# rknightion/iq-to-audio

Hardware: AMD Instinct MI355X
Metric: complex IQ MS/s end-to-end (ingest->48 kHz audio) (higher is better)
Workload: dtype i8; 1 GPU; BASELINE config 2: synthetic 60 s @ 10 MS/s int16 I/Q, 1 NFM channel, +25 kHz, bw 12.5 kHz, D=104, 6401 taps, chunk 4194304; frames_per_gpu=600000000, parallelism=1 independent capture(s), one per GPU; RCCL gather of 48 kHz audio only, audio_samples_48k=2879996, mix_sign=1, settle_steps=55

## Files before the change

iq-to-audio_amd/csrc/channelize_ring.hip:

```cpp
#include "mfma_common.h"

#include <atomic>
#include <mutex>
#include <cmath>
#include <type_traits>

namespace iqa {

typedef __attribute__((address_space(3))) void ring_lds_t;

constexpr int RG_WAVES = 8;

constexpr int RG_MAX_KS = 16;
constexpr int RG_ROWS_MAX_KS_C = 11;
constexpr int RG_W = 512;
constexpr int RG_GUARD = 64;
constexpr int RG_AS = RG_W + RG_GUARD;
constexpr int RG_ACC_BYTES = 2 * RG_AS * 8;
constexpr int RG_EMIT_WAVE = 2;
constexpr int RG_EMIT_LAG = 3;
constexpr unsigned int RG_PACE_AHEAD = 2;
constexpr int RG_PACE_SPINS = 20000;
constexpr int RG_PACE_WORDS = 16384;
constexpr int RG_PAIR_IDLE = 1 << 28;
constexpr int RG_LOADERS_MAX_KS = 13;
constexpr int RG_ROUNDS_MAX = 5;
constexpr int RG_PAIR_ROUNDS = 3;
constexpr int RG_PD = 2;

__device__ __forceinline__ void ring_dma16(const void *src, ring_lds_t *dst)
{
#if defined(__HIP_DEVICE_COMPILE__)
    __builtin_amdgcn_global_load_lds(src, dst, 16, 0, 0);
#else
    (void)src;
    (void)dst;
#endif
}

__device__ __forceinline__ unsigned lds_addr(const void *p)
{
    return static_cast<unsigned>(reinterpret_cast<size_t>((__attribute__((address_space(3))) const void *)p));
}

template <int KS, bool ROWS, bool U8 = false, bool PAIR = false>
struct RingGeo {
    static_assert(ROWS || !U8, "uint8 captures use row-staged slots");
    static_assert(!PAIR || (!ROWS && !U8), "lane pairs: contiguous slots only");
    static constexpr int TPR = PAIR ? 1 : 2;
    static constexpr int ACCS = PAIR ? 2 : 1;
    static constexpr int KBYTES = U8 ? 32 : 64;
    static constexpr int PITCH = KBYTES * KS + 16;
    static constexpr bool PADDED = KS <= 13;
    static constexpr int NI = 2 * KS + 1;
    static constexpr int UNITS_ROW = PITCH / 16;
    static constexpr int NI_ROWS = (32 * UNITS_ROW + 63) / 64;
    static constexpr int SLOT_RAW = ROWS ? (32 * PITCH > 1024 * NI_ROWS ? 32 * PITCH : 1024 * NI_ROWS) : 1024 * NI;
    static constexpr bool LOADERS = (!PAIR && (ROWS || KS <= RG_LOADERS_MAX_KS)) || (PAIR && KS <= 13);
    static constexpr bool SPLIT = LOADERS && !U8;
    static constexpr int PLANE_PITCH = 32 * KS + 16;
    static constexpr int SPLIT_F = PAIR ? 3 : 2;
    static constexpr int NLOADERS = SPLIT ? 4 : (LOADERS ? 2 : 0);
    static constexpr int SLOT = SPLIT ? 64 * PLANE_PITCH : SLOT_RAW;
    static constexpr int NDMA = ROWS ? NI_ROWS : (LOADERS ? NI : KS + 1);
    static constexpr int FIT = (160 * 1024 - ACCS * RG_ACC_BYTES) / (TPR * SLOT);
    static constexpr int RMAX = 63 / NDMA + 2;
    static constexpr int R0 = FIT < RMAX ? FIT : RMAX;
    static constexpr int RCAP = PAIR ? RG_PAIR_ROUNDS : RG_ROUNDS_MAX;
    static constexpr int R = SPLIT ? 2 : R0 > RCAP ? RCAP : (R0 < 2 ? 2 : R0);
    static constexpr int THREADS = (RG_WAVES + NLOADERS) * kWave;
    static constexpr int LDS_BYTES = R * TPR * SLOT + ACCS * RG_ACC_BYTES;
    static_assert(LDS_BYTES <= 160 * 1024, "ring + window exceed LDS");
    static_assert((R - 2) * NDMA <= 63, "vmcnt is a 6-bit counter");
};

struct RingCtx {
    char *smem;
    int *s_acc;
    const char *stream0;
    long long tile_bytes, i0, m0;
    int tiles, rounds, cnt, lane_off, rt, cp, col, h, lane;
    int row_units, pitch_units;
    int tshift;
    int half_last;
};

__device__ __forceinline__ int ring_src_off(int idx, int lane, int row_units, int pitch_units)
{
    const int q = 64 * idx + lane;
    int r = q / pitch_units;
    int u = q - r * pitch_units;
    if (r > 31) {
        r = 31;
        u = row_units - 1;
    }
    return (r * row_units + min(u, row_units - 1)) * 16;
}

struct RingEmit {
    double wc, ws;
};

struct RingEmitRegs {
    double v_re, v_im;
    double2 pr;
    int i;
};

template <bool ACC64, bool EARLY>
__device__ __forceinline__ void ring_emit_load(const MfmaArgs &a, const RingCtx &c, int k, RingEmitRegs &g)
{
    const int pos = 64 * k + 1 + c.lane;
    g.i = pos - MF_Q;
    const int s = pos & (RG_W - 1);
    if constexpr (ACC64) {
        long long *acc = reinterpret_cast<long long *>(c.s_acc);
        long long sr = acc[s], si = acc[RG_AS + s];
        if (s < RG_GUARD) {
            sr += acc[RG_W + s];
            si += acc[RG_AS + RG_W + s];
            acc[RG_W + s] = 0;
            acc[RG_AS + RG_W + s] = 0;
        }
        acc[s] = 0;
        acc[RG_AS + s] = 0;
        const int s2r = static_cast<int>(sr), s2i = static_cast<int>(si);
        const long long s1r = (sr - s2r) >> 32, s1i = (si - s2i) >> 32;
        g.v_re = static_cast<double>(s1r) * 256.0 + static_cast<double>(s2r);
        g.v_im = static_cast<double>(s1i) * 256.0 + static_cast<double>(s2i);
    } else {
        int *acc = c.s_acc;
        int sr = acc[s], si = acc[RG_AS + s];
        if (s < RG_GUARD) {
            sr += acc[RG_W + s];
            si += acc[RG_AS + RG_W + s];
            acc[RG_W + s] = 0;
            acc[RG_AS + RG_W + s] = 0;
        }
        acc[s] = 0;
        acc[RG_AS + s] = 0;
        g.v_re = static_cast<double>(sr);
        g.v_im = static_cast<double>(si);
    }
    g.pr = make_double2(0.0, 0.0);
    if constexpr (EARLY) {
        if (a.partial_in != nullptr && g.i >= 0 && g.i < c.cnt) g.pr = a.partial_in[c.i0 + g.i];
    }
}

template <bool EARLY>
__device__ __forceinline__ void ring_emit_store(const MfmaArgs &a, const RingCtx &c, RingEmit &e, const RingEmitRegs &g)
{
    const int i = g.i;
    if (i >= 0 && i < c.cnt) {
        double d_re = mfma_scaled_sum(g.v_re, a.c_re, a.unit);
        double d_im = mfma_scaled_sum(g.v_im, a.c_im, a.unit);
        if (a.partial_in != nullptr) {
            const double2 pr = EARLY ? g.pr : a.partial_in[c.i0 + i];
            d_re = __dadd_rn(d_re, pr.x);
            d_im = __dadd_rn(d_im, pr.y);
        }
        if (!a.finalize) {
            if (a.raw_partials)
                reinterpret_cast<int2 *>(a.partial_out)[c.i0 + i] = make_int2(static_cast<int>(g.v_re), static_cast<int>(g.v_im));
            else
                a.partial_out[c.i0 + i] = make_double2(d_re, d_im);
        } else {
            a.out[c.i0 + i] = mfma_finish(d_re, d_im, a.conj_sum, a.rotate, e.wc, e.ws, a.sc_re, a.sc_im);
        }
    }
    const double nc = e.wc * a.rot64_re - e.ws * a.rot64_im;
    e.ws = fma(e.wc, a.rot64_im, e.ws * a.rot64_re);
    e.wc = nc;
}

template <bool ACC64>
__device__ __forceinline__ void ring_emit_group(const MfmaArgs &a, const RingCtx &c, RingEmit &e, int k)
{
    RingEmitRegs g;
    ring_emit_load<ACC64, false>(a, c, k, g);
    ring_emit_store<false>(a, c, e, g);
}

template <int KS, bool ROWS, bool U8, bool PAIR = false>
__device__ __forceinline__ void ring_wait_and_barrier(int younger)
{
    using G = RingGeo<KS, ROWS, U8, PAIR>;
    constexpr int R = G::R, N = G::NDMA;
    if (R >= 5 && younger == 3) asm volatile("s_waitcnt vmcnt(%0)\n\ts_barrier" ::"n"(R >= 5 ? 3 * N : 0) : "memory");
    else if (R >= 4 && younger == 2) asm volatile("s_waitcnt vmcnt(%0)\n\ts_barrier" ::"n"(R >= 4 ? 2 * N : 0) : "memory");
    else if (R >= 3 && younger == 1) asm volatile("s_waitcnt vmcnt(%0)\n\ts_barrier" ::"n"(R >= 3 ? N : 0) : "memory");
    else asm volatile("s_waitcnt vmcnt(0)\n\ts_barrier" ::: "memory");
}

template <int KS, bool ACC64>
__device__ __forceinline__ void ring_loader(const MfmaArgs &a, const RingCtx &c)
{
    using G = RingGeo<KS, true, true>;
    constexpr int R = G::R, SLOT = G::SLOT;
    const int cp = c.cp;
    int soff[G::NI_ROWS];
    const int row_bytes = static_cast<int>(c.tile_bytes >> 5);
#pragma unroll
    for (int i = 0; i < G::NI_ROWS; ++i) {
        const int q = 64 * i + c.lane;
        int r = q / G::UNITS_ROW;
        int u = q - r * G::UNITS_ROW;
        if (r > 31) {
            r = 31;
            u = G::UNITS_ROW - 2;
        }
        soff[i] = r * row_bytes + min(u, G::UNITS_ROW - 2) * 16;
    }
    auto issue_tile = [&](int tile, int slot) {
        const char *src = c.stream0 + static_cast<long long>(min(tile, c.tiles - 1)) * c.tile_bytes;
        char *dst = c.smem + (slot * 2 + cp) * SLOT;
#pragma unroll
        for (int i = 0; i < G::NI_ROWS; ++i)
            ring_dma16(src + soff[i], (ring_lds_t *)(dst + i * 1024));
    };
#pragma unroll
    for (int rr = 0; rr < R - 1; ++rr) issue_tile(2 * rr + cp, rr);
    RingEmit em{1.0, 0.0};
    double st_re = a.rot64_re * a.rot64_re - a.rot64_im * a.rot64_im, st_im = 2.0 * a.rot64_re * a.rot64_im;
    if (a.finalize && a.rotate) {
        const unsigned long long m = static_cast<unsigned long long>(c.m0 + (64 * cp + 1 + c.lane - MF_Q));
        const unsigned long long ph = a.rot_base + m * a.rot_step;
        sincospi(2.0 * (static_cast<double>(ph >> 11) * (1.0 / 9007199254740992.0)), &em.ws, &em.wc);
    }
    MfmaArgs a2 = a;
    a2.rot64_re = st_re;
    a2.rot64_im = st_im;
    int slot = 0;
    for (int r = 0; r < c.rounds; ++r) {
        ring_wait_and_barrier<KS, true, true>(min(R - 2, c.rounds - 1 - r));
        if (r + R - 1 < c.rounds) issue_tile(2 * (r + R - 1) + cp, (slot == 0) ? R - 1 : slot - 1);
        if (r >= RG_EMIT_LAG && ((r - RG_EMIT_LAG) & 1) == cp) {
            asm volatile("" ::: "memory");
            ring_emit_group<ACC64>(a2, c, em, r - RG_EMIT_LAG);
            asm volatile("" ::: "memory");
        }
        slot = (slot + 1 == R) ? 0 : slot + 1;
    }
    asm volatile("s_waitcnt vmcnt(0) lgkmcnt(0)\n\ts_barrier" ::: "memory");
    const int k_last = (c.cnt + 62) >> 6;
    for (int k = max(c.rounds - RG_EMIT_LAG, 0); k <= k_last; ++k)
        if ((k & 1) == cp) ring_emit_group<ACC64>(a2, c, em, k);
}

struct __attribute__((packed, aligned(4))) ring_raw16 {
    int x, y, z, w;
};

template <int KS, bool ACC64, bool ROWS, int HALF, bool PAIR = false>
__device__ __forceinline__ void ring_loader_split(const MfmaArgs &a, const RingCtx &c)
{
    constexpr bool EMITTER = PAIR ? HALF < 2 : HALF == 0;
    constexpr bool UNEVEN = !PAIR && KS >= 12;
    constexpr int P0 = KS >= 12 ? KS - 2 : KS;
    constexpr int STRIDE = PAIR ? RingGeo<KS, ROWS, false, PAIR>::NLOADERS : 2;
    constexpr int NP = UNEVEN ? (HALF ? 2 * KS - P0 : P0) : (2 * KS + STRIDE - 1) / STRIDE;
    auto piece = [](int j) { return UNEVEN ? (HALF ? P0 + j : j) : STRIDE * j + HALF; };
    using G = RingGeo<KS, ROWS, false, PAIR>;
    constexpr int SLOT = G::SLOT, PP = G::PLANE_PITCH, F = G::SPLIT_F;
    const int cp = c.cp;
    const int upr = ROWS ? 4 * KS : c.row_units;
    const int row_bytes = static_cast<int>(c.tile_bytes >> 5);
    constexpr bool TABLE = KS <= 8;
    int doff[TABLE ? NP : 1], soff[TABLE ? NP : 1];
    unsigned rowu[TABLE ? 1 : (NP + 1) / 2];
    if constexpr (!TABLE) {
#pragma unroll
        for (int j = 0; j < (NP + 1) / 2; ++j) rowu[j] = 0;
    }
#pragma unroll
    for (int j = 0; j < NP; ++j) {
        const int q = 64 * piece(j) + c.lane;
        const int row = q / upr, u = q - row * upr;
        if constexpr (TABLE) {
            doff[j] = row < 32 ? row * PP + 8 * u : -1;
            soff[j] = row < 32 ? row * row_bytes + 16 * u : 31 * row_bytes + 16 * (upr - 1);
        } else {
            const unsigned f = row < 32 ? static_cast<unsigned>((row << 6) | u) : static_cast<unsigned>((31 << 6) | (upr - 1) | (1 << 11));
            rowu[j >> 1] |= f << (16 * (j & 1));
        }
    }
    int4 buf[F][NP];
    auto request = [&](int round, auto set) {
        constexpr int S = decltype(set)::value;
        const char *src = c.stream0 + static_cast<long long>(PAIR ? min(round, c.rounds - 1) : min(2 * round + cp, c.tiles - 1)) * c.tile_bytes;
#pragma unroll
        for (int j = 0; j < NP; ++j) {
            int so;
            if constexpr (TABLE) so = soff[j];
            else {
                const unsigned f = rowu[j >> 1] >> (16 * (j & 1));
                so = static_cast<int>((f >> 6) & 31u) * row_bytes + 16 * static_cast<int>(f & 63u);
            }
            const ring_raw16 t = *reinterpret_cast<const ring_raw16 *>(src + so);
            buf[S][j] = make_int4(t.x, t.y, t.z, t.w);
        }
    };
    auto stage = [&](int slot, auto set) {
        constexpr int S = decltype(set)::value;
        char *hi0 = c.smem + (PAIR ? slot : slot * 2 + cp) * SLOT;
#pragma unroll
        for (int j = 0; j < NP; ++j) {
            const int4 d = buf[S][j];
            int2 hi, lo;
            hi.x = __builtin_amdgcn_perm(d.y, d.x, 0x07050301);
            hi.y = __builtin_amdgcn_perm(d.w, d.z, 0x07050301);
            lo.x = __builtin_amdgcn_perm(d.y, d.x, 0x06040200) ^ 0x80808080;
            lo.y = __builtin_amdgcn_perm(d.w, d.z, 0x06040200) ^ 0x80808080;
            int dq;
            if constexpr (TABLE) dq = doff[j];
            else {
                const unsigned f = rowu[j >> 1] >> (16 * (j & 1));
                dq = (f & 2048u) ? -1 : static_cast<int>((f >> 6) & 31u) * PP + 8 * static_cast<int>(f & 63u);
            }
            if (dq >= 0) {
                *reinterpret_cast<int2 *>(hi0 + dq) = hi;
                *reinterpret_cast<int2 *>(hi0 + 32 * PP + dq) = lo;
            }
        }
    };
    request(0, std::integral_constant<int, 0>{});
    stage(0, std::integral_constant<int, 0>{});
    request(1, std::integral_constant<int, 1 % F>{});
    request(2, std::integral_constant<int, 2 % F>{});
    if constexpr (F == 3) request(3, std::integral_constant<int, 0>{});
    static_assert(F == 2 || F == 3, "the prologue and the unrolled loop below are written for two or three rounds in flight");
    RingEmit em{1.0, 0.0};
    double st_re = a.rot64_re * a.rot64_re - a.rot64_im * a.rot64_im, st_im = 2.0 * a.rot64_re * a.rot64_im;
    if (EMITTER && a.finalize && a.rotate) {
        const unsigned long long m = static_cast<unsigned long long>(c.m0 + ((PAIR ? 0 : 64 * cp) + 1 + c.lane - MF_Q));
        const unsigned long long ph = a.rot_base + m * a.rot_step;
        sincospi(2.0 * (static_cast<double>(ph >> 11) * (1.0 / 9007199254740992.0)), &em.ws, &em.wc);
    }
    MfmaArgs a2 = a;
    if constexpr (!PAIR) {
        a2.rot64_re = st_re;
        a2.rot64_im = st_im;
    }
    auto group_of = [&](int r) {
        if constexpr (PAIR) {
            const int re = r - c.tshift, lag = 5 + cp;
            return (re >= lag && ((re - lag) & 1) == 0) ? (re - lag) >> 1 : -1;
        } else {
            return (r >= RG_EMIT_LAG && ((r - RG_EMIT_LAG) & 1) == cp) ? r - RG_EMIT_LAG : -1;
        }
    };
    constexpr bool PR_AHEAD = PAIR || KS <= 11;
    double2 pr_next = make_double2(0.0, 0.0);
    auto round_body = [&](int r, auto set) {
        asm volatile("s_waitcnt lgkmcnt(0)\n\ts_barrier" ::: "memory");
        if (r + 1 < c.rounds) stage((r + 1) & 1, set);
        const double2 pr_now = pr_next;
        if (PR_AHEAD && EMITTER && a.partial_in != nullptr) {
            const int kn = group_of(r + 1);
            if (kn >= 0) {
                const int i = 64 * kn + 1 + c.lane - MF_Q;
                pr_next = (i >= 0 && i < c.cnt) ? a.partial_in[c.i0 + i] : make_double2(0.0, 0.0);
            }
        }
        request(r + 1 + F, set);
        const int k = EMITTER ? group_of(r) : -1;
        if (k >= 0) {
            asm volatile("" ::: "memory");
            if constexpr (PR_AHEAD) {
                RingEmitRegs g;
                ring_emit_load<ACC64, false>(a2, c, k, g);
                g.pr = pr_now;
                ring_emit_store<true>(a2, c, em, g);
            } else {
                ring_emit_group<ACC64>(a2, c, em, k);
            }
            asm volatile("" ::: "memory");
        }
    };
    int r = 0;
    if constexpr (F == 3) {
        for (; r + 3 <= c.rounds; r += 3) {
            round_body(r, std::integral_constant<int, 1>{});
            round_body(r + 1, std::integral_constant<int, 2>{});
            round_body(r + 2, std::integral_constant<int, 0>{});
        }
        if (r < c.rounds) {
            round_body(r, std::integral_constant<int, 1>{});
            if (r + 1 < c.rounds) round_body(r + 1, std::integral_constant<int, 2>{});
        }
    } else {
        for (; r + 2 <= c.rounds; r += 2) {
            round_body(r, std::integral_constant<int, 1>{});
            round_body(r + 1, std::integral_constant<int, 0>{});
        }
        if (r < c.rounds) round_body(r, std::integral_constant<int, 1>{});
    }
    asm volatile("s_waitcnt vmcnt(0) lgkmcnt(0)\n\ts_barrier" ::: "memory");
    if constexpr (EMITTER) {
        const int k_last = (c.cnt + 62) >> 6;
        if constexpr (PAIR) {
            const int own = c.rounds - c.tshift, lag = 5 + cp;
            const int k_next = own > lag ? ((own - 1 - lag) >> 1) + 1 : 0;
            if (c.tshift < RG_PAIR_IDLE)
                for (int k = k_next; k <= k_last; ++k) ring_emit_group<ACC64>(a2, c, em, k);
        } else {
            for (int k = max(c.rounds - RG_EMIT_LAG, 0); k <= k_last; ++k)
                if ((k & 1) == cp) ring_emit_group<ACC64>(a2, c, em, k);
        }
    }
}

template <int KS, bool ACC64, bool ROWS, bool U8, bool ISSUER, bool EMIT, bool DEFER, bool PAIR, typename SKIPT, bool HALF = false>
__device__ __forceinline__ void ring_main(const MfmaArgs &a, const RingCtx &c, const v4i_t (&fq)[KS][2], SKIPT)
{
    constexpr int SKIP = SKIPT::value;
    using G = RingGeo<KS, ROWS, U8, PAIR>;
    constexpr int R = G::R, SLOT = G::SLOT;
    static_assert(!(ROWS && ISSUER), "row-staged slots are always fed by loader waves");
    const int RG_EMIT_LAG_PAIR = 5 + c.cp;
    const int rt = c.rt, cp = c.cp;
    int soff[(ISSUER && G::PADDED) ? KS + 1 : 1];
    if constexpr (ISSUER && G::PADDED) {
#pragma unroll
        for (int i = 0; i <= KS; ++i) soff[i] = ring_src_off(min(2 * i + (rt & 1), 2 * KS), c.lane, c.row_units, c.pitch_units);
    } else {
        soff[0] = c.lane * 16;
    }
    const int odd_kib = (rt & 1) * 1024;
    auto issue = [&](int tile, int slot, int i) {
        const char *tile0 = c.stream0 + static_cast<long long>(min(tile, (PAIR ? c.rounds : c.tiles) - 1)) * c.tile_bytes;
        char *slot0 = c.smem + (PAIR ? slot : slot * 2 + cp) * SLOT;
        const int at = (i < KS) ? odd_kib + i * 2048 : 2 * KS * 1024;
        if constexpr (ISSUER && G::PADDED) {
            ring_dma16(tile0 + soff[i], (ring_lds_t *)(slot0 + at));
        } else {
            ring_dma16(tile0 + soff[0] + at, (ring_lds_t *)(slot0 + at));
        }
    };
    if (ISSUER) {
#pragma unroll
        for (int rr = 0; rr < R - 1; ++rr)
#pragma unroll
            for (int i = 0; i <= KS; ++i) issue(PAIR ? rr : 2 * rr + cp, rr, i);
    }
    RingEmit em{1.0, 0.0};
    if (EMIT && a.finalize && a.rotate) {
        const unsigned long long m = static_cast<unsigned long long>(c.m0 + (1 + c.lane - MF_Q));
        const unsigned long long ph = a.rot_base + m * a.rot_step;
        sincospi(2.0 * (static_cast<double>(ph >> 11) * (1.0 / 9007199254740992.0)), &em.ws, &em.wc);
    }
    const v16i_t zero16 = {0, 0, 0, 0, 0, 0, 0, 0, 0, 0, 0, 0, 0, 0, 0, 0};
    auto scatter = [&](int t, const v16i_t &acc1, const v16i_t &acc2) {
        const int slot_idx = ((t * 32 + c.col + 4 * c.h + 1) & (RG_W - 1)) + (rt >> 1) * RG_AS + (rt & 1) * 32;
        if constexpr (ACC64) {
            const unsigned p = lds_addr(reinterpret_cast<long long *>(c.s_acc) + slot_idx);
#pragma unroll
            for (int q = 0; q < 16; ++q) {
                const long long comb = (static_cast<long long>(acc1[q]) << 32) + static_cast<long long>(acc2[q]);
                const int off = 8 * ((q & 3) + 8 * (q >> 2));
                asm volatile("ds_add_u64 %0, %1 offset:%2" ::"v"(p), "v"(comb), "n"(off));
            }
        } else {
            const unsigned p = lds_addr(c.s_acc + slot_idx);
#pragma unroll
            for (int q = 0; q < 16; ++q) {
                const int comb = (acc1[q] << 8) + acc2[q];
                const int off = 4 * ((q & 3) + 8 * (q >> 2));
                asm volatile("ds_add_u32 %0, %1 offset:%2" ::"v"(p), "v"(comb), "n"(off));
            }
        }
    };
    constexpr bool DEFER_ADDS = DEFER && !G::SPLIT;
    v16i_t held1 = zero16, held2 = zero16;
    int held_t = -1;
    int slot = 0;
    bool pace_on = PAIR && a.pace != nullptr && a.pace_units > 1 && c.rounds < 8000;
    for (int r = 0; r < c.rounds; ++r) {
        if (ISSUER) ring_wait_and_barrier<KS, ROWS, U8, PAIR>(min(R - 2, c.rounds - 1 - r));
        else asm volatile("s_barrier" ::: "memory");
        if constexpr (PAIR && !ISSUER && !EMIT && !DEFER) {
            if (c.rt == 3 && c.cp == 0 && pace_on && (r & 1) == 0) {
                const unsigned int mine = static_cast<unsigned int>(r >> 1);
                if (c.lane == 0) __hip_atomic_store(a.pace + a.pace_slot, (a.pace_token << 12) | mine, __ATOMIC_RELAXED, __HIP_MEMORY_SCOPE_AGENT);
                for (int spin = 0;; ++spin) {
                    unsigned int q = mine;
                    if (c.lane < a.pace_units) {
                        const unsigned int v = __hip_atomic_load(a.pace + (a.pace_slot - a.pace_slot % a.pace_units) + c.lane, __ATOMIC_RELAXED,
                                                                 __HIP_MEMORY_SCOPE_AGENT);
                        if ((v >> 12) == a.pace_token) q = v & 0xFFFu;
                    }
#pragma unroll
                    for (int o = 1; o < 16; o <<= 1) q = min(q, static_cast<unsigned int>(__shfl_xor(static_cast<int>(q), o, kWave)));
                    q = static_cast<unsigned int>(__builtin_amdgcn_readfirstlane(static_cast<int>(q)));
                    if (mine <= q + RG_PACE_AHEAD) break;
                    if (spin >= RG_PACE_SPINS) {
                        pace_on = false;
                        break;
                    }
                    __builtin_amdgcn_s_sleep(32);
                }
            }
        }
        const bool pf = ISSUER && (r + R - 1 < c.rounds);
        const int pf_tile = PAIR ? r + R - 1 : 2 * (r + R - 1) + cp;
        const int pf_slot = (slot == 0) ? R - 1 : slot - 1;
        if (pf) {
#pragma unroll
            for (int i = 0; i <= KS; ++i) issue(pf_tile, pf_slot, i);
        }
        const int re = r - c.tshift;
        const bool emit_now = EMIT && (PAIR ? (re >= RG_EMIT_LAG_PAIR && ((re - RG_EMIT_LAG_PAIR) & 1) == 0) : re >= RG_EMIT_LAG);
        RingEmitRegs eg;
        if (emit_now) {
            asm volatile("" ::: "memory");
            ring_emit_load<ACC64, true>(a, c, PAIR ? (re - RG_EMIT_LAG_PAIR) >> 1 : re - RG_EMIT_LAG, eg);
            asm volatile("" ::: "memory");
        }
        if (DEFER_ADDS && held_t >= 0) {
            scatter(held_t, held1, held2);
            held_t = -1;
        }
        bool store_pending = emit_now;
#pragma unroll
        for (int j = 0; j < 1; ++j) {
        const int t = PAIR ? re : 2 * r + cp;
        if (t >= 0 && t < c.tiles) {
            const bool store_here = store_pending;
            store_pending = false;
            const char *la = c.smem + (PAIR ? slot : slot * 2 + cp) * SLOT + c.lane_off;
            auto tile_body = [&](auto skip_low) {
                constexpr bool SKIP_LOW = decltype(skip_low)::value;
                constexpr int PD = KS < RG_PD ? KS : RG_PD;
                v16i_t acc1, acc2;
                if constexpr (U8) {
                    v4i_t du[KS];
#pragma unroll
                    for (int ks = 0; ks < PD; ++ks) du[ks] = *reinterpret_cast<const v4i_t *>(la + 32 * ks);
#pragma unroll
                    for (int ks = 0; ks < KS; ++ks) {
                        v4i_t v = du[ks];
                        v.x ^= 0x80808080;
                        v.y ^= 0x80808080;
                        v.z ^= 0x80808080;
                        v.w ^= 0x80808080;
                        if (ks + PD < KS) du[ks + PD] = *reinterpret_cast<const v4i_t *>(la + 32 * (ks + PD));
                        acc1 = __builtin_amdgcn_mfma_i32_32x32x32_i8(fq[ks][0], v, ks ? acc1 : zero16, 0, 0, 0);
                        acc2 = __builtin_amdgcn_mfma_i32_32x32x32_i8(fq[ks][1], v, ks ? acc2 : zero16, 0, 0, 0);
                    }
                } else if constexpr (G::SPLIT) {
                    v4i_t hh[KS], ll[KS];
                    constexpr bool half_last = HALF;
                    auto fetch = [&](int ks) {
                        if (ks == KS - 1 && half_last) {
                            const int2 h2 = *reinterpret_cast<const int2 *>(la - 8 * c.h + 32 * ks);
                            const int2 l2 = *reinterpret_cast<const int2 *>(la - 8 * c.h + 32 * G::PLANE_PITCH + 32 * ks);
                            hh[ks].x = h2.x;
                            hh[ks].y = h2.y;
                            ll[ks].x = l2.x;
                            ll[ks].y = l2.y;
                        } else {
                            hh[ks] = *reinterpret_cast<const v4i_t *>(la + 32 * ks);
                            ll[ks] = *reinterpret_cast<const v4i_t *>(la + 32 * G::PLANE_PITCH + 32 * ks);
                        }
                    };
#pragma unroll
                    for (int ks = 0; ks < PD; ++ks) fetch(ks);
#pragma unroll
                    for (int ks = 0; ks < KS; ++ks) {
                        const v4i_t hi = hh[ks], lo = ll[ks];
                        if (ks + PD < KS) fetch(ks + PD);
                        if (ks == KS - 1 && half_last) {
                            auto pack = [](int x, int y) { return static_cast<long>((static_cast<unsigned long long>(static_cast<unsigned>(y)) << 32) | static_cast<unsigned>(x)); };
                            const long a1 = pack(fq[ks][0].x, fq[ks][0].y), a2 = pack(fq[ks][1].x, fq[ks][1].y);
                            const long bh = pack(hi.x, hi.y), bl = pack(lo.x, lo.y);
                            acc1 = __builtin_amdgcn_mfma_i32_32x32x16_i8(a1, bh, ks ? acc1 : zero16, 0, 0, 0);
                            acc2 = __builtin_amdgcn_mfma_i32_32x32x16_i8(a1, bl, ks ? acc2 : zero16, 0, 0, 0);
                            if constexpr (!SKIP_LOW) acc2 = __builtin_amdgcn_mfma_i32_32x32x16_i8(a2, bh, acc2, 0, 0, 0);
                        } else {
                            acc1 = __builtin_amdgcn_mfma_i32_32x32x32_i8(fq[ks][0], hi, ks ? acc1 : zero16, 0, 0, 0);
                            acc2 = __builtin_amdgcn_mfma_i32_32x32x32_i8(fq[ks][0], lo, ks ? acc2 : zero16, 0, 0, 0);
                            if constexpr (!SKIP_LOW) acc2 = __builtin_amdgcn_mfma_i32_32x32x32_i8(fq[ks][1], hi, acc2, 0, 0, 0);
                        }
                    }
                } else {
                    v4i_t dd[KS][2];
#pragma unroll
                    for (int ks = 0; ks < PD; ++ks) {
                        dd[ks][0] = *reinterpret_cast<const v4i_t *>(la + 64 * ks);
                        dd[ks][1] = *reinterpret_cast<const v4i_t *>(la + 64 * ks + 16);
                    }
#pragma unroll
                    for (int ks = 0; ks < KS; ++ks) {
                        if (EMIT && ks == KS - 3 && store_here) ring_emit_store<true>(a, c, em, eg);
                        const v4i_t d0 = dd[ks][0], d1 = dd[ks][1];
                        v4i_t hi, lo;
                        hi.x = __builtin_amdgcn_perm(d0.y, d0.x, 0x07050301);
                        hi.y = __builtin_amdgcn_perm(d0.w, d0.z, 0x07050301);
                        hi.z = __builtin_amdgcn_perm(d1.y, d1.x, 0x07050301);
                        hi.w = __builtin_amdgcn_perm(d1.w, d1.z, 0x07050301);
                        lo.x = __builtin_amdgcn_perm(d0.y, d0.x, 0x06040200) ^ 0x80808080;
                        lo.y = __builtin_amdgcn_perm(d0.w, d0.z, 0x06040200) ^ 0x80808080;
                        lo.z = __builtin_amdgcn_perm(d1.y, d1.x, 0x06040200) ^ 0x80808080;
                        lo.w = __builtin_amdgcn_perm(d1.w, d1.z, 0x06040200) ^ 0x80808080;
                        if (ks + PD < KS) {
                            dd[ks + PD][0] = *reinterpret_cast<const v4i_t *>(la + 64 * (ks + PD));
                            dd[ks + PD][1] = *reinterpret_cast<const v4i_t *>(la + 64 * (ks + PD) + 16);
                        }
                        acc1 = __builtin_amdgcn_mfma_i32_32x32x32_i8(fq[ks][0], hi, ks ? acc1 : zero16, 0, 0, 0);
                        acc2 = __builtin_amdgcn_mfma_i32_32x32x32_i8(fq[ks][0], lo, ks ? acc2 : zero16, 0, 0, 0);
                        if constexpr (!SKIP_LOW) acc2 = __builtin_amdgcn_mfma_i32_32x32x32_i8(fq[ks][1], hi, acc2, 0, 0, 0);
                    }
                }
                if (DEFER_ADDS) {
                    held1 = acc1;
                    held2 = acc2;
                    held_t = t;
                } else {
                    scatter(t, acc1, acc2);
                }
            };
            if constexpr (SKIP == 2 && !U8) {
                tile_body(std::true_type{});
            } else if constexpr (SKIP == 1 && !U8) {
                if (a.high_taps_only) tile_body(std::true_type{});
                else tile_body(std::false_type{});
            } else {
                tile_body(std::false_type{});
            }
        }
        }
        if (store_pending) ring_emit_store<true>(a, c, em, eg);
        slot = (slot + 1 == R) ? 0 : slot + 1;
    }
    if (DEFER_ADDS && held_t >= 0) scatter(held_t, held1, held2);
    asm volatile("s_waitcnt vmcnt(0) lgkmcnt(0)\n\ts_barrier" ::: "memory");
    if (EMIT) {
        const int k_last = (c.cnt + 62) >> 6;
        const int own = c.rounds - c.tshift;
        const int k_next = PAIR ? (own > RG_EMIT_LAG_PAIR ? ((own - 1 - RG_EMIT_LAG_PAIR) >> 1) + 1 : 0) : max(own - RG_EMIT_LAG, 0);
        if (!PAIR || c.tshift < RG_PAIR_IDLE)
            for (int k = k_next; k <= k_last; ++k) ring_emit_group<ACC64>(a, c, em, k);
    }
}

template <int KS, bool ACC64, bool ROWS, bool U8, bool PAIR = false, bool SKIPK = false, bool HALF = false>
__device__ __forceinline__ void ring_block(const MfmaArgs &a, long long range_idx)
{
    using G = RingGeo<KS, ROWS, U8, PAIR>;
    constexpr int R = G::R, SLOT = G::SLOT;
    constexpr bool LOADERS = G::LOADERS;
    extern __shared__ __attribute__((aligned(16))) char smem[];
    const int tid = threadIdx.x;
    const int wave = __builtin_amdgcn_readfirstlane(tid >> 6);
    RingCtx c;
    c.lane = tid & 63;
    c.rt = wave & 3;
    c.cp = wave >= RG_WAVES ? (wave - RG_WAVES) & 1 : (wave >> 2) & 1;
    c.col = c.lane & 31;
    c.h = c.lane >> 5;

    c.i0 = range_idx * a.range;
    c.cnt = static_cast<int>(min(static_cast<long long>(a.range), a.n_out - c.i0));
    c.m0 = a.m_lo + c.i0;
    c.tiles = (c.cnt + 63 + 31) >> 5;
    c.rounds = PAIR ? c.tiles + a.pair_extra : (c.tiles + 1) >> 1;
    c.tshift = PAIR ? a.pair_shift : 0;
    c.smem = smem;
    c.s_acc = reinterpret_cast<int *>(smem + R * G::TPR * SLOT);
    for (int i = tid; i < G::ACCS * RG_ACC_BYTES / 4; i += G::THREADS) c.s_acc[i] = 0;
    if (PAIR) c.s_acc += c.cp * (RG_ACC_BYTES / 4);

    constexpr int FB = U8 ? 2 : 4;
    const long long row_bytes = static_cast<long long>(FB) * a.D;
    c.tile_bytes = 32 * row_bytes;
    const char *stream = reinterpret_cast<const char *>(a.raw) + FB * ((c.m0 - MF_Q - a.col_shift) * a.D + 1 - a.consumed) +
                         (ROWS ? G::KBYTES * a.k_first : 0);
    c.row_units = static_cast<int>(row_bytes >> 4);
    c.pitch_units = G::PADDED ? (c.row_units | 1) : c.row_units;
    c.lane_off = G::SPLIT ? c.col * G::PLANE_PITCH + 16 * c.h : c.col * (ROWS ? G::PITCH : 16 * c.pitch_units) + (G::KBYTES / 2) * c.h;

    if constexpr (LOADERS) {
        if (wave >= RG_WAVES) {
            c.stream0 = stream;
            __syncthreads();
            if constexpr (G::SPLIT && PAIR) {
                switch (wave - RG_WAVES) {
                    case 0: ring_loader_split<KS, ACC64, ROWS, 0, true>(a, c); break;
                    case 1: ring_loader_split<KS, ACC64, ROWS, 1, true>(a, c); break;
                    case 2: ring_loader_split<KS, ACC64, ROWS, 2, true>(a, c); break;
                    default: ring_loader_split<KS, ACC64, ROWS, 3, true>(a, c); break;
                }
            } else if constexpr (G::SPLIT) {
                if ((wave - RG_WAVES) >> 1) ring_loader_split<KS, ACC64, ROWS, 1>(a, c);
                else ring_loader_split<KS, ACC64, ROWS, 0>(a, c);
            } else {
                ring_loader<KS, ACC64>(a, c);
            }
            return;
        }
    }
    v4i_t fq[KS][2];
    {
        const v4i_t *fa = a.afrag + c.rt * 128 + c.lane;
#pragma unroll
        for (int ks = 0; ks < KS; ++ks)
#pragma unroll
            for (int pc = 0; pc < 2; ++pc) fq[ks][pc] = fa[(ks * 8 + pc) * 64];
#pragma unroll
        for (int ks = 0; ks < KS; ++ks) asm volatile("" ::"v"(fq[ks][0]), "v"(fq[ks][1]));
    }
    c.half_last = HALF;
    if constexpr (HALF) {
        static_assert(!ROWS && !U8 && !PAIR, "the half last k step exists for single lanes over contiguous byte-plane slots");
#pragma unroll
        for (int pc = 0; pc < 2; ++pc) {
            const v4i_t f = fq[KS - 1][pc];
            const int z0 = __shfl(f.z, c.lane ^ 32, kWave), w0 = __shfl(f.w, c.lane ^ 32, kWave);
            if (c.h) {
                fq[KS - 1][pc].x = z0;
                fq[KS - 1][pc].y = w0;
            }
        }
    }
    __syncthreads();
    c.stream0 = stream;
    if constexpr (PAIR && G::SPLIT) {
        constexpr int SA = SKIPK ? 2 : 0, SB = 0;
        if (c.cp) ring_main<KS, ACC64, ROWS, U8, false, false, true, true>(a, c, fq, std::integral_constant<int, SB>{});
        else ring_main<KS, ACC64, ROWS, U8, false, false, false, true>(a, c, fq, std::integral_constant<int, SA>{});
    } else if constexpr (PAIR) {
        constexpr int SA = SKIPK ? 2 : 0, SB = 0;
        if (c.cp == 0 && c.rt < 2) ring_main<KS, ACC64, ROWS, U8, true, false, false, true>(a, c, fq, std::integral_constant<int, SA>{});
        else if (c.cp == 0 && c.rt == 2) ring_main<KS, ACC64, ROWS, U8, false, true, false, true>(a, c, fq, std::integral_constant<int, SA>{});
        else if (c.cp == 1 && c.rt == 3) ring_main<KS, ACC64, ROWS, U8, false, true, false, true>(a, c, fq, std::integral_constant<int, SB>{});
        else if (c.cp) ring_main<KS, ACC64, ROWS, U8, false, false, true, true>(a, c, fq, std::integral_constant<int, SB>{});
        else ring_main<KS, ACC64, ROWS, U8, false, false, false, true>(a, c, fq, std::integral_constant<int, SA>{});
    } else if constexpr (LOADERS) {
        constexpr int S1 = SKIPK ? 1 : 0;
        if (c.cp) ring_main<KS, ACC64, ROWS, U8, false, false, true, false, std::integral_constant<int, S1>, HALF>(a, c, fq, std::integral_constant<int, S1>{});
        else ring_main<KS, ACC64, ROWS, U8, false, false, false, false, std::integral_constant<int, S1>, HALF>(a, c, fq, std::integral_constant<int, S1>{});
    } else {
        constexpr int S1 = SKIPK ? 1 : 0;
        if ((c.rt >> 1) == c.cp) {
            if (c.cp) ring_main<KS, ACC64, ROWS, U8, true, false, true, false>(a, c, fq, std::integral_constant<int, S1>{});
            else ring_main<KS, ACC64, ROWS, U8, true, false, false, false>(a, c, fq, std::integral_constant<int, S1>{});
        } else if (wave == RG_EMIT_WAVE) ring_main<KS, ACC64, ROWS, U8, false, true, false, false>(a, c, fq, std::integral_constant<int, S1>{});
        else if (c.cp) ring_main<KS, ACC64, ROWS, U8, false, false, true, false>(a, c, fq, std::integral_constant<int, S1>{});
        else ring_main<KS, ACC64, ROWS, U8, false, false, false, false>(a, c, fq, std::integral_constant<int, S1>{});
    }
}

constexpr int RG_MAX_LANES = 16;

struct RingMultiArgs {
    MfmaArgs c;
    int n_lanes;
    MfmaLane lane[RG_MAX_LANES];
};

template <int KS, bool ROWS, bool U8, bool PAIR = false, bool ACC64 = false, bool SKIPK = false, bool HALF = false>
__device__ __forceinline__ void ring_multi_block(const RingMultiArgs &m)
{
    const int idx = blockIdx.x >> 3;
    const int units = PAIR ? m.n_lanes >> 1 : m.n_lanes;
    const int wv = __builtin_amdgcn_readfirstlane(static_cast<int>(threadIdx.x >> 6));
    const int li = PAIR ? 2 * (idx % units) + (wv >= RG_WAVES ? wv & 1 : (wv >> 2) & 1) : idx % units;
    const long long range_idx = static_cast<long long>(idx / units) * 8 + (blockIdx.x & 7);
    const MfmaLane &l = m.lane[li];
    MfmaArgs a = m.c;
    a.pair_shift = a.pair_extra = 0;
    a.afrag = l.afrag;
    a.out = l.out;
    a.partial_in = l.partial_in;
    a.partial_out = l.partial_out;
    a.unit = l.unit;
    a.c_re = l.c_re;
    a.c_im = l.c_im;
    a.rot_step = l.rot_step;
    a.rot_base = l.rot_base;
    a.rot64_re = l.rot64_re;
    a.rot64_im = l.rot64_im;
    a.sc_re = l.sc_re;
    a.sc_im = l.sc_im;
    a.col_shift = l.col_shift;
    a.finalize = l.finalize;
    a.conj_sum = l.conj_sum;
    a.rotate = l.rotate;
    a.raw_partials = l.raw_partials;
    a.high_taps_only = l.high_taps_only;
    if constexpr (PAIR) {
        const MfmaLane &la = m.lane[li & ~1], &lb = m.lane[li | 1];
        const bool idle_b = lb.afrag == nullptr;
        a.pair_extra = idle_b ? 0 : (la.col_shift - lb.col_shift) >> 5;
        a.col_shift = la.col_shift;
        if (li & 1) {
            a.pair_shift = idle_b ? RG_PAIR_IDLE : a.pair_extra;
            if (idle_b) a.afrag = la.afrag;
        }
        a.pace_units = units;
        a.pace_slot = static_cast<int>(range_idx) * units + idx % units;
    }
    if (range_idx * a.range >= a.n_out) return;
    ring_block<KS, ACC64, ROWS, U8, PAIR, SKIPK, HALF>(a, range_idx);
}

template <int KS, bool ACC64 = false, bool SKIPK = false>
__global__ __launch_bounds__((RingGeo<KS, false>::THREADS), (RingGeo<KS, false>::LOADERS ? 3 : 2)) void k_channelize_mfma_s16_ring_multi(RingMultiArgs m)
{
    ring_multi_block<KS, false, false, false, ACC64, SKIPK>(m);
}

template <int KS>
__global__ __launch_bounds__((RingGeo<KS, false>::THREADS), 3) void k_channelize_mfma_s16_ring_multi_half(RingMultiArgs m)
{
    static_assert(RingGeo<KS, false>::SPLIT, "byte-plane kernels only");
    ring_multi_block<KS, false, false, false, false, false, true>(m);
}

template <int KS, bool ACC64 = false, bool SKIPK = false>
__global__ __launch_bounds__((RingGeo<KS, false, false, true>::THREADS), (RingGeo<KS, false, false, true>::LOADERS ? 3 : 2)) void k_channelize_mfma_s16_ring_pairs(RingMultiArgs m)
{
    ring_multi_block<KS, false, false, true, ACC64, SKIPK>(m);
}

template <int KS, bool SKIPK = false>
__global__ __launch_bounds__((RingGeo<KS, true>::THREADS), 3) void k_channelize_mfma_s16_ring_rows_multi(RingMultiArgs m)
{
    ring_multi_block<KS, true, false, false, false, SKIPK>(m);
}

template <int KS>
__global__ __launch_bounds__((RingGeo<KS, true, true>::THREADS), 3) void k_channelize_mfma_u8_ring_rows_multi(RingMultiArgs m)
{
    ring_multi_block<KS, true, true>(m);
}

template <typename K, typename A>
static int ring_launch_kernel(K kernel, const char *name, int threads, const A &a, unsigned blocks, size_t lds, hipStream_t stream,
                              std::atomic<unsigned long long> &done)
{
    int dev = 0;
    (void)hipGetDevice(&dev);
    const unsigned long long bit = 1ull << (dev & 63);
    if (!(done.load(std::memory_order_acquire) & bit)) {
        const hipError_t e = hipFuncSetAttribute(reinterpret_cast<const void *>(kernel), hipFuncAttributeMaxDynamicSharedMemorySize, 160 * 1024);
        if (e != hipSuccess) {
            set_error("%s: cannot raise the dynamic LDS limit on device %d: %s", name, dev, hipGetErrorString(e));
            return IQA_EHIP;
        }
        done.fetch_or(bit, std::memory_order_release);
    }
    hipLaunchKernelGGL(kernel, dim3(blocks), dim3(threads), lds, stream, a);
    return check_launch(name);
}

template <int KS>
static int ring_launch_multi(const RingMultiArgs &m, unsigned blocks, size_t lds, hipStream_t stream, bool rows, bool u8, bool acc64, bool skipk)
{
    static std::atomic<unsigned long long> done[8] = {{0}, {0}, {0}, {0}, {0}, {0}, {0}, {0}};
    if (acc64) {
        if constexpr (KS < RG_MAX_KS) {
            if (!rows && !u8) {
                if (skipk)
                    return ring_launch_kernel(k_channelize_mfma_s16_ring_multi<KS, true, true>, "k_channelize_mfma_s16_ring_multi64", RingGeo<KS, false>::THREADS, m, blocks, lds, stream, done[4]);
                return ring_launch_kernel(k_channelize_mfma_s16_ring_multi<KS, true>, "k_channelize_mfma_s16_ring_multi64", RingGeo<KS, false>::THREADS, m, blocks, lds, stream, done[3]);
            }
        }
        set_error("multi-lane launches with 64-bit sums: contiguous int16 slots, at most %d k steps (got %d)", RG_MAX_KS - 1, KS);
        return IQA_EINVAL;
    }
    if constexpr (KS <= RG_ROWS_MAX_KS_C) {
        if (u8) return ring_launch_kernel(k_channelize_mfma_u8_ring_rows_multi<KS>, "k_channelize_mfma_u8_ring_rows_multi", RingGeo<KS, true, true>::THREADS, m, blocks, lds, stream, done[2]);
        if (rows && skipk) return ring_launch_kernel(k_channelize_mfma_s16_ring_rows_multi<KS, true>, "k_channelize_mfma_s16_ring_rows_multi", RingGeo<KS, true>::THREADS, m, blocks, lds, stream, done[5]);
        if (rows) return ring_launch_kernel(k_channelize_mfma_s16_ring_rows_multi<KS>, "k_channelize_mfma_s16_ring_rows_multi", RingGeo<KS, true>::THREADS, m, blocks, lds, stream, done[1]);
    } else {
        if (u8 || rows) {
            set_error("row-staged ring kernels take at most %d k steps per pass (got %d)", RG_ROWS_MAX_KS_C, KS);
            return IQA_EINVAL;
        }
    }
    if (skipk) return ring_launch_kernel(k_channelize_mfma_s16_ring_multi<KS, false, true>, "k_channelize_mfma_s16_ring_multi", RingGeo<KS, false>::THREADS, m, blocks, lds, stream, done[6]);
    if constexpr (KS <= 8) {
        const int rem = (2 * m.c.D) & 31;
        if (rem != 0 && rem <= 16)
            return ring_launch_kernel(k_channelize_mfma_s16_ring_multi_half<KS>, "k_channelize_mfma_s16_ring_multi", RingGeo<KS, false>::THREADS, m, blocks, lds, stream, done[7]);
    }
    return ring_launch_kernel(k_channelize_mfma_s16_ring_multi<KS>, "k_channelize_mfma_s16_ring_multi", RingGeo<KS, false>::THREADS, m, blocks, lds, stream, done[0]);
}

constexpr int RG_PAIR_MIN_KS = 9;

template <int KS>
static int ring_launch_pairs(const RingMultiArgs &m, unsigned blocks, hipStream_t stream, bool acc64, bool skipk)
{
    static std::atomic<unsigned long long> done{0}, done64{0}, done_s{0}, done64_s{0};
    if constexpr (KS >= RG_PAIR_MIN_KS && KS != 15) {
        using G = RingGeo<KS, false, false, true>;
        if (acc64) {
            if constexpr (KS <= 14) {
                if (skipk)
                    return ring_launch_kernel(k_channelize_mfma_s16_ring_pairs<KS, true, true>, "k_channelize_mfma_s16_ring_pairs64", G::THREADS, m, blocks, G::LDS_BYTES, stream, done64_s);
                return ring_launch_kernel(k_channelize_mfma_s16_ring_pairs<KS, true>, "k_channelize_mfma_s16_ring_pairs64", G::THREADS, m, blocks, G::LDS_BYTES, stream, done64);
            }
            set_error("lane pairs with 64-bit sums: 9..14 k steps (got %d)", KS);
            return IQA_EINVAL;
        }
        if (skipk) return ring_launch_kernel(k_channelize_mfma_s16_ring_pairs<KS, false, true>, "k_channelize_mfma_s16_ring_pairs", G::THREADS, m, blocks, G::LDS_BYTES, stream, done_s);
        return ring_launch_kernel(k_channelize_mfma_s16_ring_pairs<KS>, "k_channelize_mfma_s16_ring_pairs", G::THREADS, m, blocks, G::LDS_BYTES, stream, done);
    } else {
        set_error("lane pairs: %d k steps not instantiated (%d..14, 16)", KS, RG_PAIR_MIN_KS);
        return IQA_EINVAL;
    }
}

static unsigned int *ring_pace_buffer(unsigned int &token, int words, hipStream_t stream)
{
    static std::mutex mu;
    static unsigned int *buf[64] = {};
    static int next_off[64] = {};
    static unsigned int next_token = 1;
    int dev = 0;
    (void)hipGetDevice(&dev);
    std::lock_guard<std::mutex> lock(mu);
    token = next_token = (next_token % 0xFFFFFu) + 1;
    unsigned int *&b = buf[dev & 63];
    if (b == nullptr) {
        hipStreamCaptureStatus st = hipStreamCaptureStatusNone;
        if (hipStreamIsCapturing(stream, &st) != hipSuccess || st != hipStreamCaptureStatusNone) {
            (void)hipGetLastError();
            return nullptr;
        }
        void *p = nullptr;
        if (hipMalloc(&p, RG_PACE_WORDS * sizeof(unsigned int)) != hipSuccess) {
            (void)hipGetLastError();
            return nullptr;
        }
        if (hipMemset(p, 0, RG_PACE_WORDS * sizeof(unsigned int)) != hipSuccess || hipDeviceSynchronize() != hipSuccess) {
            (void)hipGetLastError();
            (void)hipFree(p);
            return nullptr;
        }
        b = static_cast<unsigned int *>(p);
    }
    if (words > RG_PACE_WORDS) return nullptr;
    int &off = next_off[dev & 63];
    if (off + words > RG_PACE_WORDS) off = 0;
    unsigned int *mine = b + off;
    off += (words + 63) & ~63;
    return mine;
}

bool mfma_ring_pairs_supported(int decimation, int k_first, int k_count, bool u8, bool acc64)
{
    return mfma_ring_mode(decimation, k_first, k_count, acc64, u8) == 1 && k_count >= RG_PAIR_MIN_KS && k_count != 15 && (!acc64 || k_count <= 14);
}

constexpr int RG_ROWS_MAX_KS = RG_ROWS_MAX_KS_C;

int mfma_ring_mode(int decimation, int k_first, int k_count, bool acc64, bool u8)
{
    const int ks_all = (2 * decimation + 31) / 32;
    if (!u8 && decimation >= 4 && (decimation & 3) == 0 && ks_all <= (acc64 ? RG_MAX_KS - 1 : RG_MAX_KS) && k_first == 0 && k_count == ks_all) return 1;
    if (!acc64 && decimation >= 1 && k_count >= 1 && k_count <= RG_ROWS_MAX_KS && k_first >= 0 && k_first + k_count <= ks_all) return 2;
    return 0;
}

bool mfma_ring_supported(int decimation)
{
    const int ks = (2 * decimation + 31) / 32;
    return decimation >= 4 && (decimation & 3) == 0 && ks <= RG_MAX_KS;
}

template <int LO, int HI, class F>
static auto with_ks(int ks, F &&f)
{
    if constexpr (LO < HI) {
        if (ks > LO) return with_ks<LO + 1, HI>(ks, f);
    }
    return f(std::integral_constant<int, LO>{});
}

template <int KS>
static constexpr size_t ring_bytes_of(bool rows, bool u8)
{
    return u8     ? static_cast<size_t>(RingGeo<KS, true, true>::R) * 2 * RingGeo<KS, true, true>::SLOT + RG_ACC_BYTES
           : rows ? static_cast<size_t>(RingGeo<KS, true>::R) * 2 * RingGeo<KS, true>::SLOT + RG_ACC_BYTES
                  : static_cast<size_t>(RingGeo<KS, false>::R) * 2 * RingGeo<KS, false>::SLOT + RG_ACC_BYTES;
}

size_t mfma_ring_lds_bytes(int ksteps, bool rows, bool u8)
{
    if (ksteps < 1 || ksteps > (rows ? RG_ROWS_MAX_KS : RG_MAX_KS)) return 0;
    return with_ks<1, RG_MAX_KS>(ksteps, [&](auto k) { return ring_bytes_of<decltype(k)::value>(rows, u8); });
}

int mfma_ring_launch_multi(const MfmaArgs &a, const MfmaLane *lanes, int n_lanes, size_t lds, hipStream_t stream, bool rows, bool u8,
                           bool pairs, bool acc64)
{
    if (n_lanes < 1 || n_lanes > RG_MAX_LANES) {
        set_error("a multi-lane launch takes 1..%d lanes (got %d)", RG_MAX_LANES, n_lanes);
        return IQA_EINVAL;
    }
    if (pairs) {
        if (rows || u8 || (n_lanes & 1)) {
            set_error("lane pairs: contiguous int16 slots and an even number of lanes");
            return IQA_EINVAL;
        }
        for (int i = 0; i < n_lanes; i += 2)
            if (lanes[i].afrag == nullptr || (lanes[i + 1].afrag != nullptr && lanes[i].col_shift < lanes[i + 1].col_shift)) {
                set_error("lane pairs: lane %d must exist and have the larger (or the same) tap-row group of its pair", i);
                return IQA_EINVAL;
            }
    }
    RingMultiArgs m;
    m.c = a;
    m.n_lanes = n_lanes;
    for (int i = 0; i < n_lanes; ++i) m.lane[i] = lanes[i];
    for (int i = n_lanes; i < RG_MAX_LANES; ++i) m.lane[i] = m.lane[0];
    bool skipk = false;
    if (!u8) {
        if (pairs) {
            skipk = true;
            for (int i = 0; i < n_lanes; i += 2)
                if (!lanes[i].high_taps_only || (lanes[i + 1].afrag != nullptr && lanes[i + 1].high_taps_only)) skipk = false;
        } else {
            for (int i = 0; i < n_lanes; ++i) skipk = skipk || lanes[i].high_taps_only != 0;
        }
    }
    if (!skipk)
        for (int i = 0; i < RG_MAX_LANES; ++i) m.lane[i].high_taps_only = 0;
    const long long ranges = (a.n_out + a.range - 1) / a.range;
    const long long groups = (ranges + 7) / 8;
    const unsigned blocks = static_cast<unsigned>(groups * (pairs ? n_lanes / 2 : n_lanes) * 8);
    if (a.ksteps < 1 || a.ksteps > RG_MAX_KS) {
        set_error("ring kernel: %d k steps not instantiated (1..%d)", a.ksteps, RG_MAX_KS);
        return IQA_EINVAL;
    }
    if (pairs) {
        m.c.pace = nullptr;
        m.c.pace = ring_pace_buffer(m.c.pace_token, static_cast<int>(std::min<long long>(groups * 8 * (n_lanes / 2), RG_PACE_WORDS + 1)), stream);
        return with_ks<1, RG_MAX_KS>(a.ksteps, [&](auto k) { return ring_launch_pairs<decltype(k)::value>(m, blocks, stream, acc64, skipk); });
    }
    return with_ks<1, RG_MAX_KS>(a.ksteps, [&](auto k) {
        return ring_launch_multi<decltype(k)::value>(m, blocks, lds, stream, rows, u8, acc64, skipk);
    });
}

}
```

Before: 947,600 MS/s.

## Pre-reduce MFMA accumulator scatter with DPP lane shifts before LDS atomics

```diff
diff --git a/iq-to-audio_amd/csrc/channelize_ring.hip b/iq-to-audio_amd/csrc/channelize_ring.hip
--- a/iq-to-audio_amd/csrc/channelize_ring.hip
+++ b/iq-to-audio_amd/csrc/channelize_ring.hip
@@ -41,6 +41,22 @@
 __device__ __forceinline__ unsigned lds_addr(const void *p)
 {
     return static_cast<unsigned>(reinterpret_cast<size_t>((__attribute__((address_space(3))) const void *)p));
+}
+
+#ifndef IQA_SCATTER_PREREDUCE
+#define IQA_SCATTER_PREREDUCE 1
+#endif
+constexpr int RG_SCATTER_PRE = IQA_SCATTER_PREREDUCE;
+
+__device__ __forceinline__ int ring_shr1(int v)
+{
+    return __builtin_amdgcn_update_dpp(0, v, 0x111, 0xf, 0xf, true);
+}
+
+template <int N, int BANK>
+__device__ __forceinline__ int ring_row_top(int keep, int v)
+{
+    return __builtin_amdgcn_update_dpp(keep, v, 0x101 + N, 0xf, BANK, false);
 }
 
 template <int KS, bool ROWS, bool U8 = false, bool PAIR = false>
@@ -463,11 +479,56 @@
             }
         } else {
             const unsigned p = lds_addr(c.s_acc + slot_idx);
-#pragma unroll
-            for (int q = 0; q < 16; ++q) {
-                const int comb = (acc1[q] << 8) + acc2[q];
-                const int off = 4 * ((q & 3) + 8 * (q >> 2));
-                asm volatile("ds_add_u32 %0, %1 offset:%2" ::"v"(p), "v"(comb), "n"(off));
+            if constexpr (RG_SCATTER_PRE == 0) {
+#pragma unroll
+                for (int q = 0; q < 16; ++q) {
+                    const int comb = (acc1[q] << 8) + acc2[q];
+                    const int off = 4 * ((q & 3) + 8 * (q >> 2));
+                    asm volatile("ds_add_u32 %0, %1 offset:%2" ::"v"(p), "v"(comb), "n"(off));
+                }
+            } else {
+                int fx[4];
+#pragma unroll
+                for (int g = 0; g < 4; ++g) {
+                    int e0 = (acc1[4 * g] << 8) + acc2[4 * g], e1 = (acc1[4 * g + 1] << 8) + acc2[4 * g + 1];
+                    int e2 = (acc1[4 * g + 2] << 8) + acc2[4 * g + 2], e3 = (acc1[4 * g + 3] << 8) + acc2[4 * g + 3];
+                    asm("" : "+v"(e0), "+v"(e1), "+v"(e2), "+v"(e3));
+                    e2 += ring_shr1(e3);
+                    e1 += ring_shr1(e2);
+                    e0 += ring_shr1(e1);
+                    asm volatile("ds_add_u32 %0, %1 offset:%2" ::"v"(p), "v"(e0), "n"(32 * g));
+                    if constexpr (RG_SCATTER_PRE == 1) {
+                        fx[g] = ring_row_top<1, 0x8>(ring_row_top<0, 0x8>(e1, e2), e3);
+                    } else {
+                        if (g == 0) fx[0] = ring_row_top<1, 0x8>(ring_row_top<0, 0x8>(e1, e2), e3);
+                        if (g == 1) fx[0] = ring_row_top<5, 0x4>(ring_row_top<4, 0x4>(ring_row_top<3, 0x4>(fx[0], e1), e2), e3);
+                        if (g == 2) fx[0] = ring_row_top<9, 0x2>(ring_row_top<8, 0x2>(ring_row_top<7, 0x2>(fx[0], e1), e2), e3);
+                        if (g == 3) fx[0] = ring_row_top<13, 0x1>(ring_row_top<12, 0x1>(ring_row_top<11, 0x1>(fx[0], e1), e2), e3);
+                    }
+                }
+                const int up = 15 - (c.lane & 15);
+                unsigned long long sv;
+                if constexpr (RG_SCATTER_PRE == 1) {
+                    const unsigned pf = p + 4 * (1 + 2 * up);
+                    asm volatile("s_and_saveexec_b64 %0, %1\n\t"
+                                 "ds_add_u32 %2, %3\n\t"
+                                 "ds_add_u32 %2, %4 offset:32\n\t"
+                                 "ds_add_u32 %2, %5 offset:64\n\t"
+                                 "ds_add_u32 %2, %6 offset:96\n\t"
+                                 "s_mov_b64 exec, %0\n\t"
+                                 "s_nop 4"
+                                 : "=&s"(sv)
+                                 : "s"(0xE000E000E000E000ull), "v"(pf), "v"(fx[0]), "v"(fx[1]), "v"(fx[2]), "v"(fx[3]));
+                } else {
+                    const int top_idx = ((t * 32 + c.col + 4 * c.h + 1 + up) & (RG_W - 1)) + (rt >> 1) * RG_AS + (rt & 1) * 32;
+                    const unsigned pf = lds_addr(c.s_acc + top_idx) + 4 * (1 + (up & 3) + 8 * (up >> 2));
+                    asm volatile("s_and_saveexec_b64 %0, %1\n\t"
+                                 "ds_add_u32 %2, %3\n\t"
+                                 "s_mov_b64 exec, %0\n\t"
+                                 "s_nop 4"
+                                 : "=&s"(sv)
+                                 : "s"(0xEEEEEEEEEEEEEEEEull), "v"(pf), "v"(fx[0]));
+                }
             }
         }
     };
diff --git a/iq-to-audio_amd/csrc/probe/dpp_shift_probe.hip b/iq-to-audio_amd/csrc/probe/dpp_shift_probe.hip
--- /dev/null
+++ b/iq-to-audio_amd/csrc/probe/dpp_shift_probe.hip
@@ -0,0 +1,34 @@
+#include <hip/hip_runtime.h>
+
+template <int CTRL, int BANK, bool BOUND>
+__device__ __forceinline__ int dpp(int old, int src)
+{
+    return __builtin_amdgcn_update_dpp(old, src, CTRL, 0xf, BANK, BOUND);
+}
+
+__global__ void k_row_shr1(int *p)
+{
+    const int a = p[threadIdx.x], b = p[64 + threadIdx.x];
+    p[threadIdx.x] = a + dpp<0x111, 0xf, true>(0, b);
+}
+
+__global__ void k_wave_shr1(int *p)
+{
+    const int a = p[threadIdx.x], b = p[64 + threadIdx.x];
+    p[threadIdx.x] = a + dpp<0x138, 0xf, true>(0, b);
+}
+
+__global__ void k_gather_row_top(int *p)
+{
+    int a = p[threadIdx.x];
+    const int b = p[64 + threadIdx.x], c = p[128 + threadIdx.x];
+    a = dpp<0x101, 0x8, false>(a, b);
+    a = dpp<0x102, 0x8, false>(a, c);
+    p[threadIdx.x] = a;
+}
+
+__global__ void k_row_bcast(int *p)
+{
+    const int a = p[threadIdx.x];
+    p[threadIdx.x] = dpp<0x142, 0xf, false>(a, a) + dpp<0x143, 0xf, false>(a, a);
+}
```

After: 951,900 MS/s, median of 6. Within noise of the previous version (+0.5%).
